# rishabhgoel0213/ZeroClone

Measured on AMD Instinct MI355X. Metric: MCTS node-expansions/sec (whole node), Connect4 800 sims/move at 1/2/4/8 MI355X, higher is better.
Workload: dtype f64

## Files before the change

zeroclone_amd/csrc/c4_device.h:

```cpp
#pragma once
#include <math.h>

#include "c4_order_table.h"
#include "zc_internal.h"

namespace zc {
namespace {

__constant__ uint32_t d_order[128] = {ZC_C4_ORDER_LIST};

constexpr uint32_t kRingMask = kRingWords - 1;
constexpr uint64_t kBottom = 0x0000040810204081ull;
constexpr uint64_t kFull = kBottom * 0x3Full;
constexpr uint64_t kTop = kBottom << 5;
constexpr int kTabBytes = 128 * 4 + 128 * 8;

__device__ __forceinline__ uint32_t untried_init(uint32_t n) { return ((1u << n) - 1u) | (n << 28); }
__device__ __forceinline__ uint32_t untried_count(uint32_t u) { return (uint32_t)__popc(u & 0x7Fu); }

__device__ __forceinline__ void load_tables(uint32_t *s_order) {
    for (int i = (int)threadIdx.x; i < 128; i += blockDim.x) s_order[i] = d_order[i];
    uint8_t *const s_sel = (uint8_t *)(s_order + 128);
    for (int i = (int)threadIdx.x; i < 1024; i += blockDim.x) {
        const uint32_t m = (uint32_t)i >> 3, r = (uint32_t)i & 7u;
// ... 98 lines not shown
    m = b & (b >> 1);
    r |= m & (m >> 2);
    m = b & (b >> 6);
    r |= m & (m >> 12);
    m = b & (b >> 8);
    r |= m & (m >> 16);
    return r != 0;
}

__device__ __forceinline__ uint32_t temper(uint32_t y) {
    y ^= y >> 11;
    y ^= (y << 7) & 0x9d2c5680u;
    y ^= (y << 15) & 0xefc60000u;
    y ^= y >> 18;
    return y;
}

struct Rng {
    uint32_t *ring;
    uint32_t base;
    int32_t wrel;
    uint32_t off;
    int32_t grel;
    uint32_t wt;
    uint32_t wn;
    uint32_t wx;
    __device__ __forceinline__ int32_t use() const { return wrel + (int32_t)off; }
    __device__ __forceinline__ uint32_t slot(int32_t rel) const { return (base + (uint32_t)rel) & kRingMask; }
    __device__ __forceinline__ uint32_t cur() const { return wt; }
};

__device__ __forceinline__ int32_t rng_generate(uint32_t *ring, uint32_t base, int32_t grel, int32_t target) {
    const uint32_t lane = lane_id();
    constexpr int K = kChunk / 64;
    while (grel < target) {
        uint32_t a[K], b[K], m[K];
        const uint32_t p0 = base + (uint32_t)grel + lane;
#pragma unroll
        for (int k = 0; k < K; ++k) {
            const uint32_t p = p0 + 64u * k;
            a[k] = ring[(p - 624) & kRingMask];
            b[k] = ring[(p - 623) & kRingMask];
            m[k] = ring[(p - 227) & kRingMask];
        }
#pragma unroll
        for (int k = 0; k < K; ++k) {
            const uint32_t p = p0 + 64u * k;
            const uint32_t y = (a[k] & 0x80000000u) | (b[k] & 0x7fffffffu);
            ring[p & kRingMask] = m[k] ^ (y >> 1) ^ ((b[k] & 1u) ? 0x9908b0dfu : 0u);
        }
        grel += kChunk;
        wave_mem_order();
    }
    return grel;
}

__device__ __forceinline__ void rng_fill(Rng &r, int32_t target) {
    if (r.grel < target) r.grel = rng_generate(r.ring, r.base, r.grel, target);
}

__device__ __forceinline__ void rng_open(Rng &r, uint32_t *ring, uint64_t use0, uint64_t gen0) {
    r.ring = ring;
    r.base = (uint32_t)use0;
    r.grel = (int32_t)(gen0 - use0);
    r.off = (uint32_t)use0 & (uint32_t)(kWin - 1);
    r.wrel = -(int32_t)r.off;
    rng_fill(r, r.wrel + 3 * kWin);
    r.wt = temper(r.ring[r.slot(r.wrel + (int32_t)lane_id())]);
    r.wn = temper(r.ring[r.slot(r.wrel + kWin + (int32_t)lane_id())]);
    r.wx = r.ring[r.slot(r.wrel + 2 * kWin + (int32_t)lane_id())];
    vmem_ready(r.wx);
}

__device__ __forceinline__ void rng_advance(Rng &r) {
    r.wrel += kWin;
    r.off -= (uint32_t)kWin;
    r.wt = r.wn;
    r.wn = temper(r.wx);
    if (r.grel < r.wrel + 3 * kWin) rng_fill(r, r.wrel + 3 * kWin);
    r.wx = r.ring[r.slot(r.wrel + 2 * kWin + (int32_t)lane_id())];
    vmem_ready(r.wx);
}

template <class R>
__device__ __forceinline__ uint32_t rng_view(const R &r) {
    const uint32_t j = lane_id() + r.off;
    const int idx = (int)(j << 2);
    const uint32_t a = (uint32_t)__builtin_amdgcn_ds_bpermute(idx, (int)r.wt);
    const uint32_t b = (uint32_t)__builtin_amdgcn_ds_bpermute(idx, (int)r.wn);
    return j < 64u ? a : b;
}

__device__ __forceinline__ void rng_close(const Rng &r, uint64_t use0, uint64_t *rngpos) {
    rngpos[0] = use0 + (uint64_t)(int64_t)r.use();
    rngpos[1] = use0 + (uint64_t)(int64_t)r.grel;
}

constexpr int kLRingWords = 1024;
constexpr uint32_t kLRingMask = kLRingWords - 1;
constexpr int kLRingBytes = kLRingWords * 4;

struct LRng {
    uint32_t *lds;
    uint32_t base;
    int32_t wrel;
    uint32_t off;
    int32_t hrel;
    uint32_t wa, wb, ph;
    __device__ __forceinline__ uint32_t cur() const { return ph ? wb : wa; }
    uint32_t wx;
    uint32_t ia, ib, im;
    __device__ __forceinline__ int32_t use() const { return wrel + (int32_t)off; }
    __device__ __forceinline__ uint32_t slot(int32_t rel) const { return (base + (uint32_t)rel) & kLRingMask; }
};

__device__ __forceinline__ uint32_t mt_twist(uint32_t a, uint32_t b, uint32_t m) {
    const uint32_t y = (a & 0x80000000u) | (b & 0x7fffffffu);
    return m ^ (y >> 1) ^ ((b & 1u) ? 0x9908b0dfu : 0u);
}

__device__ __forceinline__ void lrng_prefetch(LRng &r) {
    const int32_t p = r.wrel + 192 + (int32_t)lane_id();
    r.ia = r.lds[r.slot(p - 624)];
    r.ib = r.lds[r.slot(p - 623)];
    r.im = r.lds[r.slot(p - 227)];
}

__device__ __forceinline__ void lrng_generate_abs(uint32_t *lds, uint64_t g, uint64_t end) {
    const uint32_t lane = lane_id();
    for (; g < end; g += 64) {
        const uint32_t p = (uint32_t)g + lane;
        const uint32_t a = lds[(p - 624) & kLRingMask], b = lds[(p - 623) & kLRingMask],
                       m = lds[(p - 227) & kLRingMask];
        if (g + lane < end) lds[p & kLRingMask] = mt_twist(a, b, m);
        wave_mem_order();
    }
}

__device__ __forceinline__ void lrng_open(LRng &r, uint32_t *lds, const uint32_t *ring, uint64_t use0, uint64_t gen0) {
    const uint32_t lane = lane_id();
    r.lds = lds;
    r.base = (uint32_t)use0;
    r.off = (uint32_t)use0 & (uint32_t)(kWin - 1);
    r.wrel = -(int32_t)r.off;
    const uint64_t w0 = use0 - r.off, target = w0 + 192;
    const uint64_t g = gen0 <= w0 + 960 ? gen0 : (target < 624 ? 624 : target);
    for (uint32_t i = lane; i < (uint32_t)kLRingWords; i += 64) {
        const uint32_t p = (uint32_t)g - (uint32_t)kLRingWords + i;
        lds[p & kLRingMask] = ring[p & kRingMask];
    }
    wave_mem_order();
    lrng_generate_abs(lds, g, target);
    r.hrel = (int32_t)(g - use0);
    r.wa = temper(lds[r.slot(r.wrel + (int32_t)lane)]);
    r.wb = temper(lds[r.slot(r.wrel + kWin + (int32_t)lane)]);
    r.ph = 0;
    r.wx = lds[r.slot(r.wrel + 2 * kWin + (int32_t)lane)];
    lrng_prefetch(r);
}

__device__ __forceinline__ uint32_t rng_view(const LRng &r) {
    const uint32_t j = lane_id() + r.off;
    const int idx = (int)(j << 2);
    const uint32_t a = (uint32_t)__builtin_amdgcn_ds_bpermute(idx, (int)r.wa);
    const uint32_t b = (uint32_t)__builtin_amdgcn_ds_bpermute(idx, (int)r.wb);
    return (j ^ r.ph) < 64u ? a : b;
}

__device__ __forceinline__ void rng_advance(LRng &r) {
    r.wrel += kWin;
    r.off -= (uint32_t)kWin;
    const uint32_t t = temper(r.wx);
    if (r.ph) r.wb = t;
    else r.wa = t;
    r.ph ^= 64u;
    const int32_t p = r.wrel + 128 + (int32_t)lane_id();
    uint32_t x = mt_twist(r.ia, r.ib, r.im);
    if (r.wrel + 128 < r.hrel) {
        const uint32_t old = r.lds[r.slot(p)];
        x = p < r.hrel ? old : x;
    }
    r.lds[r.slot(p)] = x;
    r.wx = x;
    lrng_prefetch(r);
}

__device__ __forceinline__ void lrng_skip(LRng &r, uint32_t w) {
    r.off += w;
    while (r.off >= (uint32_t)kWin) rng_advance(r);
}

__device__ __forceinline__ void lrng_close(const LRng &r, uint32_t *ring, uint64_t use0, uint64_t *rngpos) {
    const uint32_t lane = lane_id();
    const uint64_t U = use0 + (uint64_t)(int64_t)r.use();
    uint64_t G = use0 + (uint64_t)(int64_t)max(r.wrel + 192, r.hrel);
    const uint64_t blk = U ? (U - 1) / 624 : 0;
    const uint64_t bend = (blk + 1) * 624;
    wave_mem_order();
    if (G < bend) {
        lrng_generate_abs(r.lds, G, bend);
        G = bend;
    }
    const uint64_t wu = U & ~(uint64_t)(kWin - 1);
    uint64_t start = wu < blk * 624 ? wu : blk * 624;
    start = start < G - 624 ? start : G - 624;
    for (uint64_t q = start + lane; q < G; q += 64) ring[(uint32_t)q & kRingMask] = r.lds[(uint32_t)q & kLRingMask];
    if (lane == 0) {
        rngpos[0] = U;
        rngpos[1] = G;
    }
}

template <class R>
__device__ __forceinline__ uint32_t rng_below(R &r, uint32_t n) {
    const uint32_t sh = (uint32_t)__clz(n);
    const uint32_t lane = lane_id();
    for (;;) {
        if (r.off >= (uint32_t)kWin) rng_advance(r);
        const uint32_t v = r.cur() >> sh;
        const uint64_t bal = __ballot((v | ((lane - r.off) & 0x80000000u)) < n);
        if (bal) {
            const int f = __builtin_ctzll(bal);
            r.off = (uint32_t)f + 1;
            return (uint32_t)__builtin_amdgcn_readlane((int)v, f);
        }
        r.off = kWin;
    }
}

template <class R>
__device__ __forceinline__ uint32_t rng_below_pick(R &r, uint32_t n, const uint8_t *row) {
    const uint32_t sh = (uint32_t)__clz(n);
    const uint32_t lane = lane_id();
    for (;;) {
        if (r.off >= (uint32_t)kWin) rng_advance(r);
        const uint32_t v = r.cur() >> sh;
        const uint32_t pick = row[v & 7u];
        const uint64_t bal = __ballot((v | ((lane - r.off) & 0x80000000u)) < n);
        if (bal) {
            const int f = __builtin_ctzll(bal);
            r.off = (uint32_t)f + 1;
            return (uint32_t)__builtin_amdgcn_readlane((int)pick, f);
        }
        r.off = kWin;
    }
}

struct Counters {
    int32_t expansions = 0, depth_sum = 0, plies = 0, blocks = 0;
    __device__ __forceinline__ void add(int32_t &c, int32_t v) { c += (lane_id() == 0) ? v : 0; }
};

struct Leaf {
    uint64_t p0, p1;
    uint32_t meta;
    int32_t val;
    uint32_t ow;
    uint32_t pad;
};

struct Fresh {
    uint32_t u;
    uint32_t ow;
    uint32_t link;
    uint32_t lmask;
    int32_t na;
    int32_t w;
    uint32_t pad1, pad2;
    uint16_t ch[8];
};
static_assert(sizeof(Fresh) == 48, "Fresh is three 16-byte LDS slots");

struct Tree {
    uint8_t *nodes;
    __device__ __forceinline__ uint8_t *rec(int nd) const { return nodes + (size_t)nd * kRecBytes; }
    __device__ __forceinline__ uint32_t *hdr(int nd) const { return (uint32_t *)rec(nd); }
    __device__ __forceinline__ uint16_t *child(int nd) const { return (uint16_t *)(rec(nd) + 16); }
    __device__ __forceinline__ int32_t *na(int nd) const { return (int32_t *)(rec(nd) + 32); }
    __device__ __forceinline__ double *q(int nd) const { return (double *)(rec(nd) + 64); }
    __device__ __forceinline__ int32_t *w(int nd) const { return (int32_t *)(rec(nd) + 64); }
};

__device__ __forceinline__ void node_init(const Tree &t, int nd, int parent, int pact, int depth, uint32_t ow) {
    const uint32_t lane = lane_id();
    const uint32_t n = (ow >> 24) & 15u;
    if (lane == 0) {
        uint4 h;
        h.x = 0;
        h.y = untried_init(n);
        h.z = (uint32_t)(parent & 0xFFFF) | ((uint32_t)(pact & 0xFF) << 16) | ((uint32_t)depth << 24);
        h.w = ow;
        *(uint4 *)t.rec(nd) = h;
    }
    if (lane < kSlots) {
        t.child(nd)[lane] = 0xFFFF;
        t.na(nd)[lane] = 0;
        t.q(nd)[lane] = 0.0;
    }
}

__device__ __forceinline__ bool valid_state(uint64_t p0, uint64_t p1, int turn) {
    if ((p0 & p1) || ((p0 | p1) & ~kFull) || (turn & ~1)) return false;
    const uint64_t occ = p0 | p1;
#pragma unroll
    for (int c = 0; c < 7; ++c) {
        const uint64_t col = (occ >> (7 * c)) & 0x3Full;
        if (col & (col + 1)) return false;
    }
    return true;
}

template <bool ON>
struct Stamp {
    uint64_t ph[kPhases];
    uint64_t t;
    __device__ __forceinline__ Stamp() : t(ON ? __builtin_amdgcn_s_memtime() : 0) {
        for (int i = 0; i < kPhases; ++i) ph[i] = 0;
    }
    __device__ __forceinline__ void mark(int k) {
        if (ON) {
            const uint64_t now = __builtin_amdgcn_s_memtime();
            ph[k] += now - t;
            t = now;
        }
    }
};

using ConstDouble = const __attribute__((address_space(4))) double;

struct FlushSel {
    int f0;
    int x0node, d0;
    uint32_t ppath;
    bool x0_dirty;
    uint32_t x_u, x_ch;
    bool planned = false;
// ... 262 lines not shown
```

zeroclone_amd/csrc/c4_search.hip:

```cpp
#include "c4_device.h"
#include "counter_rng.h"

namespace zc {
namespace {


__device__ __forceinline__ uint64_t readlane64(uint64_t x, int l) {
    return ((uint64_t)(uint32_t)__builtin_amdgcn_readlane((int)(x >> 32), l) << 32) |
           (uint64_t)(uint32_t)__builtin_amdgcn_readlane((int)x, l);
}

__device__ __forceinline__ uint32_t mbcnt(uint64_t m) {
    return __builtin_amdgcn_mbcnt_hi((uint32_t)(m >> 32), __builtin_amdgcn_mbcnt_lo((uint32_t)m, 0u));
}

__device__ __forceinline__ uint32_t scan_add32(uint32_t x) {
    x += (uint32_t)__builtin_amdgcn_update_dpp(0, (int)x, 0x111, 0xF, 0xF, false);
    x += (uint32_t)__builtin_amdgcn_update_dpp(0, (int)x, 0x112, 0xF, 0xF, false);
    x += (uint32_t)__builtin_amdgcn_update_dpp(0, (int)x, 0x114, 0xF, 0xF, false);
    x += (uint32_t)__builtin_amdgcn_update_dpp(0, (int)x, 0x118, 0xF, 0xF, false);
    x += (uint32_t)__builtin_amdgcn_update_dpp(0, (int)x, 0x142, 0xA, 0xF, false);
    x += (uint32_t)__builtin_amdgcn_update_dpp(0, (int)x, 0x143, 0xC, 0xF, false);
    return x;
}

__device__ __forceinline__ void scan_or16x2(uint32_t &x, uint32_t &y) {
    x |= (uint32_t)__builtin_amdgcn_update_dpp(0, (int)x, 0x111, 0xF, 0xF, false);
    y |= (uint32_t)__builtin_amdgcn_update_dpp(0, (int)y, 0x111, 0xF, 0xF, false);
    x |= (uint32_t)__builtin_amdgcn_update_dpp(0, (int)x, 0x112, 0xF, 0xF, false);
    y |= (uint32_t)__builtin_amdgcn_update_dpp(0, (int)y, 0x112, 0xF, 0xF, false);
    x |= (uint32_t)__builtin_amdgcn_update_dpp(0, (int)x, 0x114, 0xF, 0xF, false);
    y |= (uint32_t)__builtin_amdgcn_update_dpp(0, (int)y, 0x114, 0xF, 0xF, false);
    x |= (uint32_t)__builtin_amdgcn_update_dpp(0, (int)x, 0x118, 0xF, 0xF, false);
    y |= (uint32_t)__builtin_amdgcn_update_dpp(0, (int)y, 0x118, 0xF, 0xF, false);
}

__device__ __forceinline__ uint64_t in_vgpr(uint64_t x) {
    __asm__("" : "+v"(x));
    return x;
}
__device__ __forceinline__ uint32_t ff1(uint64_t m) {
    uint32_t r;
    __asm__("s_ff1_i32_b64 %0, %1" : "=s"(r) : "s"(m));
    return r;
}

#ifndef ZC_RV
#define ZC_RV 0
#endif
#ifndef ZC_LAG_MODE
#define ZC_LAG_MODE 3
#endif
__device__ __forceinline__ void set_prio(int lvl) {
    if (lvl >= 3) __builtin_amdgcn_s_setprio(3);
    else if (lvl == 2) __builtin_amdgcn_s_setprio(2);
    else if (lvl == 1) __builtin_amdgcn_s_setprio(1);
    else __builtin_amdgcn_s_setprio(0);
}
#ifndef ZC_RSTAMP
#define ZC_RSTAMP 0
#endif
#define RMARK(k)                                                    \
    do {                                                            \
        if (ZC_RSTAMP && sub) {                                     \
            __builtin_amdgcn_sched_barrier(0);                      \
            const uint64_t now_ = __builtin_amdgcn_s_memtime();     \
            __builtin_amdgcn_sched_barrier(0);                      \
            if (ZC_RSTAMP == (k)) *sub += now_ - t_;                \
            t_ = now_;                                              \
        }                                                           \
    } while (0)
template <class R>
__device__ void c4_rollouts(Leaf *L, int nb, R &rng, const uint32_t *s_order, Counters &cn,
                            uint64_t *sub = nullptr) {
    uint64_t t_ = ZC_RSTAMP && sub ? __builtin_amdgcn_s_memtime() : 0;
    const uint32_t lane = lane_id();
    const uint32_t lrow = lane >> 4;
    const bool first_row = (lrow & 1u) == 0;
    const uint32_t d1 = lrow < 2 ? 1u : 6u, d2 = lrow < 2 ? 7u : 8u;
    const uint32_t pairbits = lane < 49u ? (1u << (lane / 7u)) | (1u << (lane % 7u)) : 0u;
    for (int g = 0; g < nb; g += 64) {
      uint32_t lm_v = 0, ow_v = 0, hp_v = 0;
      int room_v = 0;
      {
        const int jj = g + (int)lane;
        if (jj < nb) {
            lm_v = L[jj].meta;
            ow_v = L[jj].ow;
            const uint64_t x0 = L[jj].p0, x1 = L[jj].p1;
            const uint64_t op_v = (lm_v >> 24) & 1u ? x0 : x1;
            room_v = has_four(op_v) ? -2 : 41 - __popcll(x0 | x1);
            const uint64_t oc = x0 | x1;
            for (int c = 0; c < 7; ++c) hp_v |= (uint32_t)__popcll((oc >> (7 * c)) & 0x3Full) << (4 * c);
        }
      }
      const int jend = min(nb, g + 64);
      for (int j = g; j < jend; ++j) {
        RMARK(6);
        const int jl = j - g;
        const uint32_t lm = (uint32_t)__builtin_amdgcn_readlane((int)lm_v, jl);
        const uint32_t tnv = (lm >> 24) & 1u;
        const uint64_t *const pp = &L[j].p0;
        uint64_t me = in_vgpr(pp[tnv]);
        uint64_t op = in_vgpr(pp[tnv ^ 1u]);
        uint32_t hp = (uint32_t)__builtin_amdgcn_readlane((int)hp_v, jl);
        const uint32_t low0 = (uint32_t)__builtin_amdgcn_readlane((int)ow_v, jl);
        const int room0 = __builtin_amdgcn_readlane(room_v, jl);
        const bool won = room0 == -2;
        int val = 0;
        int q = 0;
        RMARK(1);
        if (won) {
            val = -1;
        } else if (room0 >= 0) {
            int room = room0;
            int mask = (int)(lm >> 25);
            uint32_t ow = low0;
            uint32_t n = (ow >> 24) & 15u;
            uint32_t sh = (uint32_t)__builtin_clz(n);
            uint32_t owp = s_order[(uint32_t)mask & ~pairbits];
            for (;;) {
                RMARK(6);
                uint32_t wv, v;
                uint64_t A;
                if (rng.off >= (uint32_t)kWin) rng_advance(rng);
                wv = rng_view(rng);
                v = wv >> sh;
                A = __ballot(v < n);
                if (__builtin_expect(A == 0ull, 0)) {
                    do {
                        rng.off += (uint32_t)kWin;
                        rng_advance(rng);
                        wv = rng_view(rng);
                        v = wv >> sh;
                        A = __ballot(v < n);
                    } while (A == 0ull);
                }
#ifndef ZC_DIAG_WASTE
                cn.add(cn.blocks, 1);
#endif
                RMARK(2);
                const uint32_t cap_r = min((uint32_t)room, 30u);
                uint32_t qk = mbcnt(A);
                uint32_t col = (ow >> (3 * v)) & 7u;
                uint32_t one = mask_sel0(A, 1u << (4 * col));
                uint32_t sc = scan_add32(one);
                uint32_t row = ((sc - one + hp) >> (4 * col)) & 15u;
                uint32_t nacc = (uint32_t)__popcll(A);
                uint64_t F = __ballot(row == 5u);
                uint64_t E0 = A & (F | __ballot(qk >= min(cap_r, nacc - 1u)));
                uint32_t l0 = (uint32_t)__builtin_ctzll(E0);
                const uint64_t G = A & F & __ballot(qk < cap_r);
#if !(ZC_RV & 1)
                uint32_t lf = 64u;
                uint32_t cf = 0;
                RMARK(3);
                if (ff1(G) == l0) {
                    lf = l0;
                    cf = (uint32_t)__builtin_amdgcn_readlane((int)col, (int)lf);
                    const uint32_t ow2 = (uint32_t)__builtin_amdgcn_readlane((int)owp, (int)(8u * cf));
                    const uint32_t n2 = (ow2 >> 24) & 15u;
                    const uint32_t v2 = wv >> __clz(n2);
                    const uint64_t low = (2ull << lf) - 1ull;
                    A = (A & low) | (__ballot(v2 < n2) & ~low);
                    qk = mbcnt(A);
                    col = mask_sel(low, (ow2 >> (3 * v2)) & 7u, col);
                    one = mask_sel0(A, 1u << (4 * col));
                    sc = scan_add32(one);
                    row = ((sc - one + hp) >> (4 * col)) & 15u;
                    nacc = (uint32_t)__popcll(A);
                    F = __ballot(row == 5u) & ~low;
                    E0 = A & (F | __ballot(qk >= min(cap_r, nacc - 1u)));
                    l0 = (uint32_t)__builtin_ctzll(E0);
                }
                RMARK(4);
                const uint32_t c = ((qk & 1u) << 4) | ((qk >> 1) & 15u) | (qk & 32u);
                const uint32_t b = __umul24(col, 7u) + row;
                const uint32_t pl = (uint32_t)__builtin_amdgcn_ds_permute((int)(mask_sel(A, 63u, c) << 2), (int)b);
                const uint32_t pb = __builtin_amdgcn_permlane32_swap(pl, pl, false, false)[0];
                const uint64_t bit = 1ull << (pb & 63u);
                uint32_t blo = (uint32_t)bit, bhi = (uint32_t)(bit >> 32);
                scan_or16x2(blo, bhi);
                const uint64_t mine = ((uint64_t)bhi << 32) | blo;
                const uint64_t bd = (first_row ? me : op) | mine;
                const uint64_t m1 = bd & (bd >> d1), m2 = bd & (bd >> d2);
                const uint64_t f4 = (m1 & (m1 >> (2 * d1))) | (m2 & (m2 >> (2 * d2)));
                const uint64_t W = __ballot(f4 != 0ull);
                const uint32_t W32 = (uint32_t)W | (uint32_t)(W >> 32);
                const uint64_t Ew = A & __ballot(((W32 >> (c & 31u)) & 1u) != 0u);
#else
                uint32_t lf = 64u;
                uint32_t cf = 0;
                auto win_test = [&](uint64_t A_, uint32_t qk_, uint32_t col_, uint32_t row_, uint64_t &mine_) {
                    const uint32_t c = ((qk_ & 1u) << 4) | ((qk_ >> 1) & 15u) | (qk_ & 32u);
                    const uint32_t b = __umul24(col_, 7u) + row_;
                    const uint32_t pl = (uint32_t)__builtin_amdgcn_ds_permute((int)(mask_sel(A_, 63u, c) << 2), (int)b);
                    const uint32_t pb = __builtin_amdgcn_permlane32_swap(pl, pl, false, false)[0];
                    const uint64_t bit = 1ull << (pb & 63u);
                    uint32_t blo = (uint32_t)bit, bhi = (uint32_t)(bit >> 32);
                    scan_or16x2(blo, bhi);
                    mine_ = ((uint64_t)bhi << 32) | blo;
                    const uint64_t bd = (first_row ? me : op) | mine_;
                    const uint64_t m1 = bd & (bd >> d1), m2 = bd & (bd >> d2);
                    const uint64_t f4 = (m1 & (m1 >> (2 * d1))) | (m2 & (m2 >> (2 * d2)));
                    const uint64_t W = __ballot(f4 != 0ull);
                    const uint32_t W32 = (uint32_t)W | (uint32_t)(W >> 32);
                    return A_ & __ballot(((W32 >> (c & 31u)) & 1u) != 0u);
                };
                uint64_t Ew1 = 0, mine1 = 0;
                RMARK(3);
                if (ff1(G) == l0) {
                    lf = l0;
                    cf = (uint32_t)__builtin_amdgcn_readlane((int)col, (int)lf);
                    const uint32_t ow2 = (uint32_t)__builtin_amdgcn_readlane((int)owp, (int)(8u * cf));
                    const uint32_t n2 = (ow2 >> 24) & 15u;
                    const uint32_t v2 = wv >> __clz(n2);
                    const uint64_t low = (2ull << lf) - 1ull;
                    if (ZC_RV & 1) Ew1 = win_test(A, qk, col, row, mine1) & low;
                    A = (A & low) | (__ballot(v2 < n2) & ~low);
                    qk = mbcnt(A);
                    col = mask_sel(low, (ow2 >> (3 * v2)) & 7u, col);
                    one = mask_sel0(A, 1u << (4 * col));
                    sc = scan_add32(one);
                    row = ((sc - one + hp) >> (4 * col)) & 15u;
                    nacc = (uint32_t)__popcll(A);
                    F = __ballot(row == 5u) & ~low;
                    E0 = A & (F | __ballot(qk >= min(cap_r, nacc - 1u)));
                    l0 = (uint32_t)__builtin_ctzll(E0);
                }
                RMARK(4);
                uint64_t mine, Ew;
                if ((ZC_RV & 1) && Ew1 != 0ull) {
                    Ew = Ew1;
                    mine = mine1;
                } else {
                    Ew = win_test(A, qk, col, row, mine);
                }
#endif
                const uint32_t ew = ff1(Ew);
                const uint32_t endlane = min(ew, l0);
                const bool win = ew <= l0;
                const uint32_t endply = (uint32_t)__builtin_amdgcn_readlane((int)qk, (int)endlane);
                rng.off += endlane + 1u;
#ifdef ZC_DIAG_WASTE
                cn.add(cn.blocks, lf < 64u && endlane < lf ? 1 : 0);
                cn.add(cn.plies, lf < 64u ? 1 : 0);
#endif
                room -= (int)endply + 1;
                RMARK(5);
                if (win) {
                    val = ((room0 - room) & 1) ? 1 : -1;
                    break;
                }
                if (room < 0) {
                    val = 0;
                    break;
                }
                {
                    const uint64_t s2 = readlane64(mine, (int)((endply + 31u) >> 1));
                    const uint64_t a2 = me | readlane64(mine, (int)(endply >> 1));
                    const uint64_t b2 = op | (endply ? s2 : 0ull);
                    const bool odd = endply & 1u;
                    me = odd ? a2 : b2;
                    op = odd ? b2 : a2;
                }
                hp += (uint32_t)__builtin_amdgcn_readlane((int)sc, (int)endlane);
                const bool fa = endlane >= lf;
                const bool fe = (F >> endlane) & 1u;
                {
                    const uint32_t ce = fe ? (uint32_t)__builtin_amdgcn_readlane((int)col, (int)endlane) : cf;
                    const uint32_t ca = fa ? cf : ce;
                    const bool ff = fa | fe;
                    mask = ff ? mask & ~((1 << ca) | (1 << ce)) : mask;
                    const uint32_t ownew = (uint32_t)__builtin_amdgcn_readlane((int)owp, (int)((7u * ca + ce) & 63u));
                    ow = ff ? ownew : ow;
                    owp = s_order[(uint32_t)mask & ~pairbits];
                }
                n = (ow >> 24) & 15u;
                sh = (uint32_t)__builtin_clz(n);
            }
            q = room0 - room;
        }
        L[j].val = val;
#ifndef ZC_DIAG_WASTE
        cn.add(cn.plies, q);
#endif
      }
    }
}

__device__ void c4_rollouts_philox(Leaf *L, int nb, const uint8_t *s_sel, uint2 key, uint32_t leaf0, uint32_t tag,
                                   uint32_t game, Counters &cn) {
    const uint32_t lane = lane_id();
    for (int base = 0; base < nb; base += kBlock) {
        const int j = base + (int)lane;
        int val = 0, q = 0;
        if (j < nb) {
            const uint64_t x0 = L[j].p0, x1 = L[j].p1;
            const bool tn = (L[j].meta >> 24) & 1u;
            uint64_t me = tn ? x1 : x0;
            uint64_t op = tn ? x0 : x1;
            int stones = __popcll(me | op);
            if (has_four(op)) {
                val = -1;
            } else if (stones < 42) {
                uint32_t legal = (uint32_t)legal_mask(me | op);
                const uint4 sd = philox(make_uint4(leaf0 + (uint32_t)j, tag, game, 0x0C4F0A57u), key);
                Xoshiro128 x{sd.x | ((sd.x | sd.y | sd.z | sd.w) == 0u), sd.y, sd.z, sd.w};
                for (;;) {
                    const uint32_t n = (uint32_t)__popc(legal);
                    const uint32_t k = __umulhi(x.next(), n);
                    const uint32_t col = s_sel[legal * 8u + k];
                    const uint32_t h = (uint32_t)__popcll(((me | op) >> (7u * col)) & 0x3Full);
                    me |= 1ull << (7u * col + h);
                    ++q;
                    ++stones;
                    if (h == 5u) legal &= ~(1u << col);
                    if (has_four(me)) {
                        val = (q & 1) ? 1 : -1;
                        break;
                    }
                    if (stones == 42) {
                        val = 0;
                        break;
                    }
                    const uint64_t t = me;
                    me = op;
                    op = t;
                }
            }
            L[j].val = val;
        }
        int tot = q;
        for (int o = 32; o > 0; o >>= 1) tot += __shfl_xor(tot, o);
        cn.add(cn.plies, tot);
    }
}

struct ChainNode {
    uint64_t p0, p1;
    uint32_t ow;
    uint32_t info;
    uint32_t ul;
    uint32_t pad;
};
static_assert(sizeof(ChainNode) == 32, "chain table entry");

__device__ __forceinline__ uint64_t lanes_in(int lo, int hi) {
    const uint64_t below_hi = hi >= 64 ? ~0ull : (1ull << hi) - 1ull;
    return below_hi & ~((1ull << lo) - 1ull);
}

__device__ __forceinline__ WalkEnd walk_hbm_prefetch(const Tree &t, ConstDouble *logtab, uint64_t rp0, uint64_t rp1,
                                                     int rturn, int done, double c, int &status) {
    const uint32_t lane = lane_id();
    const uint32_t k = lane & 7u, cs = lane >> 3;
    int node = 0, depth = 0, turn = rturn, nN = done;
    uint64_t b0 = rp0, b1 = rp1;
    uint32_t pathv = (lane == 0) ? 0x00FF0000u : 0u;
    const uint8_t *R0 = t.rec(0);
    uint32_t u = uni(((const uint32_t *)R0)[1]), ow = uni(((const uint32_t *)R0)[3]);
    uint32_t ch = ((const uint16_t *)(R0 + 16))[k];
    int32_t na = ((const int32_t *)(R0 + 32))[k];
    int32_t wa = ((const int32_t *)(R0 + 64))[k];
    for (;;) {
        if (untried_count(u)) break;
        if (depth >= kMaxDepth - 2) {
            status = ZC_STATUS_INTERNAL;
            u = 0;
            break;
// ... 714 lines not shown
                        uint8_t *R = t.rec(f0 + r);
                        if (slot == 0) *(uint4 *)R = make_uint4(0u, F.u, F.link, F.ow);
                        ((uint16_t *)(R + 16))[slot] = c;
                        ((int32_t *)(R + 32))[slot] = na;
                        ((int32_t *)(R + 64))[slot] = w;
                    }
                }
            }
        }
        wave_mem_order();
        stamp.mark(6);
        done += nb;
        if (stop && done < p.sims && status == 0 && uni(spent) >= budget) break;
        if (ZC_LAG_MODE >= 2 && progress) {
            const int64_t own = ((int64_t)mv * p.sims + done) * p.n_games, avg = (int64_t)spent * p.sims;
            const int64_t mvn = (int64_t)p.sims * p.n_games;
            if (ZC_LAG_MODE == 4)
                lag = own >= avg ? 0 : own + mvn / 2 > avg ? 1 : own + mvn > avg ? 2 : 3;
            else
                lag = own < avg ? (ZC_LAG_MODE == 3 && own + mvn <= avg ? 2 : ZC_LAG_MODE == 3 ? 1 : 2) : 0;
            set_prio(lag);
        }
    }
    done_io = done;
    nnodes_io = nnodes;
    if (lagp) *lagp = lag;
    if (STAMP && lane == 0)
        for (int k_ = 0; k_ < kPhases; ++k_) p.a.phase[kPhases * (size_t)g + k_] += (int64_t)stamp.ph[k_];
}

__device__ __forceinline__ int best_column(const Tree &t, int &na_col) {
    const uint32_t lane = lane_id();
    const uint32_t k = lane & 7u;
    const uint32_t u = uni(t.hdr(0)[1]);
    const uint32_t ow = uni(t.hdr(0)[3]);
    const uint32_t nm = u >> 28;
    int bv = (k < nm) ? t.na(0)[k] : -1;
    int bi = (int)k;
    argmax8(bv, bi);
    const int best = uni(bi);
    int pos = -1;
    for (uint32_t s = 0; s < nm; ++s)
        if (((ow >> (3 * s)) & 7u) == lane) pos = (int)s;
    na_col = pos >= 0 ? t.na(0)[pos] : 0;
    return (int)((ow >> (3 * best)) & 7u);
}

template <bool STAMP, bool PHILOX, int WALK>
__device__ __forceinline__ void search_games(const SearchParams &p, uint8_t *s_dyn) {
    const SearchLds L = search_lds(s_dyn, p.bs);
    load_tables(L.s_order);
    __syncthreads();

    const uint32_t lane = lane_id();
    const int gl = (int)(blockIdx.x * (blockDim.x >> 6) + (threadIdx.x >> 6));
    if (gl >= p.n_games) return;
    const int g = p.game_ids ? uni(p.game_ids[gl]) : p.first_game + gl;
    {
        const zc_c4_state root = p.roots[gl];
        const uint64_t rp0 = uni64(root.stones[0]), rp1 = uni64(root.stones[1]);
        const int rturn = uni(root.turn);
        if (!valid_state(rp0, rp1, rturn) || legal_mask(rp0 | rp1) == 0) {
            if (lane == 0) {
                zc_game_stats st{};
                st.status = valid_state(rp0, rp1, rturn) ? ZC_STATUS_NO_MOVES : ZC_STATUS_BAD_STATE;
                p.out_stats[gl] = st;
                p.out_move[gl] = -1;
            }
            if (lane < 7) p.out_na[(size_t)gl * 7 + lane] = 0;
            return;
        }
    }
    const Arena &a = p.a;
    const Tree t{a.nodes + (size_t)g * p.M * kRecBytes};
    LRng rng;
    const uint64_t use0 = uni64(a.rngpos[2 * (size_t)g]);
    lrng_open(rng, L.ring, a.ring + (size_t)g * kRingWords, use0, uni64(a.rngpos[2 * (size_t)g + 1]));
    Counters cn;
    int status = 0, done = 0, nnodes = 1;
    search_move<STAMP, PHILOX, WALK>(p, L, gl, g, t, rng, uni((uint32_t)use0), cn, status, done, nnodes);
    int na_col;
    const int col = best_column(t, na_col);
    if (lane < 7) p.out_na[(size_t)gl * 7 + lane] = na_col;
    if (lane == 0) {
        p.out_move[gl] = col;
        zc_game_stats st{};
        st.status = status;
        st.expansions = cn.expansions;
        st.depth_sum = cn.depth_sum;
        st.leaves = p.sims;
        st.rollout_plies = cn.plies;
        st.rollout_blocks = cn.blocks;
        st.rng_words = rng.use();
        p.out_stats[gl] = st;
    }
    lrng_close(rng, a.ring + (size_t)g * kRingWords, use0, a.rngpos + 2 * (size_t)g);
}

template <bool STAMP, bool PHILOX>
__global__ __launch_bounds__(kSearchWaves * kBlock, 4) void c4_search_kernel(SearchParams p) {
    extern __shared__ __attribute__((aligned(16))) uint8_t s_dyn[];
    search_games<STAMP, PHILOX, 0>(p, s_dyn);
}

template <int WALK>
__global__ __launch_bounds__(kSearchWaves * kBlock, 4) void c4_walk_kernel(SearchParams p) {
    extern __shared__ __attribute__((aligned(16))) uint8_t s_dyn[];
    search_games<false, false, WALK>(p, s_dyn);
}

template <bool PHILOX>
__global__ __launch_bounds__(kSearchWaves * kBlock, 4) void c4_selfplay_kernel(SearchParams p) {
    extern __shared__ __attribute__((aligned(16))) uint8_t s_dyn[];
    const SearchLds L = search_lds(s_dyn, p.bs);
    load_tables(L.s_order);
    __syncthreads();

    const uint32_t lane = lane_id();
    const int gl = (int)(blockIdx.x * (blockDim.x >> 6) + (threadIdx.x >> 6));
    if (gl >= p.n_games) return;
    const int g = p.first_game + gl;
    const Arena &a = p.a;
    const Tree t{a.nodes + (size_t)g * p.M * kRecBytes};
    LRng rng;
    const uint64_t use0 = uni64(a.rngpos[2 * (size_t)g]);
    lrng_open(rng, L.ring, a.ring + (size_t)g * kRingWords, use0, uni64(a.rngpos[2 * (size_t)g + 1]));
    Counters cn;
    int status = 0;
    int finished = 0;
    int mv = 0;
    int64_t leaves = 0;
    uint64_t t_start = 0, t_last = 0;
    if (p.tstamps) t_start = t_last = __builtin_amdgcn_s_memrealtime();
    int lag = 0;
    uint4 cy = a.carry[g];
    cy = make_uint4(uni(cy.x), uni(cy.y), uni(cy.z), 0u);
    bool resume = cy.x != 0;
    for (; mv < p.moves; ++mv) {
        if (p.ticket && !resume) {
            int tk = 0;
            if (lane == 0) tk = atomicAdd(p.ticket, 1);
            if (uni(tk) >= p.budget) break;
        }
        if (p.tstamps) t_last = __builtin_amdgcn_s_memrealtime();
        zc_c4_state root = p.roots[gl];
        uint64_t s0 = uni64(root.stones[0]), s1 = uni64(root.stones[1]);
        int turn = uni(root.turn);
        if (!valid_state(s0, s1, turn) || legal_mask(s0 | s1) == 0) {
            status = ZC_STATUS_BAD_STATE;
            break;
        }
        int done = resume ? (int)cy.x : 0, nnodes = resume ? (int)cy.y : 1;
        const uint32_t tag = resume ? cy.z : uni((uint32_t)(use0 + (uint64_t)(int64_t)rng.use()));
        const int done0 = done;
        if (ZC_LAG_MODE == 1 && p.progress) {
            const int32_t tot = __hip_atomic_load(p.progress, __ATOMIC_RELAXED, __HIP_MEMORY_SCOPE_AGENT);
            lag = (int64_t)mv * p.n_games < (int64_t)uni(tot) ? 2 : 0;
            set_prio(lag);
        }
        search_move<false, PHILOX>(p, L, gl, g, t, rng, tag, cn, status, done, nnodes, p.carry ? p.ticket : nullptr,
                                   p.budget, &lag, ZC_LAG_MODE ? p.progress : nullptr, mv);
        if (ZC_LAG_MODE && p.progress && lane == 0) atomicAdd(p.progress, 1);
        leaves += done - done0;
        if (done < p.sims) {
            if (lane == 0) a.carry[g] = make_uint4((uint32_t)done, (uint32_t)nnodes, tag, 0u);
            break;
        }
        if (resume && lane == 0) a.carry[g] = make_uint4(0u, 0u, 0u, 0u);
        resume = false;
        int na_col;
        const int col = best_column(t, na_col);
        const uint64_t bit = drop_bit(s0 | s1, col);
        if (turn) s1 |= bit; else s0 |= bit;
        const bool won = has_four(turn ? s1 : s0);
        turn ^= 1;
        const int r = won ? turn * 2 - 1 : ((s0 | s1) == kFull ? 0 : ZC_C4_ONGOING);
        const size_t o = (size_t)mv * p.n_games + gl;
        if (lane == 0) {
            zc_c4_state post;
            post.stones[0] = s0;
            post.stones[1] = s1;
            post.turn = turn;
            post.reserved = 0;
            p.out_states[o] = post;
            p.out_moves16[o] = (int16_t)col;
            p.out_results[o] = r;
            p.io_roots[gl] = r == ZC_C4_ONGOING ? post : zc_c4_state{{0, 0}, 0, 0};
        }
        finished += r != ZC_C4_ONGOING;
        wave_mem_order();
    }
    if (p.ticket && lane == 0) atomicMax(p.ticket + 1, mv);
    if (p.tstamps && lane == 0) {
        uint64_t *ts = p.tstamps + 4 * (size_t)g;
        ts[0] = t_start;
        ts[1] = t_last;
        ts[2] = __builtin_amdgcn_s_memrealtime();
        const uint32_t hw = (uint32_t)__builtin_amdgcn_s_getreg(4 | (15 << 11)) |
                            ((uint32_t)__builtin_amdgcn_s_getreg(20 | (3 << 11)) << 16);
        ts[3] = (uint64_t)mv | ((uint64_t)hw << 32);
    }
    for (int k = mv + (int)lane; k < p.moves; k += kBlock) {
        const size_t o = (size_t)k * p.n_games + gl;
        p.out_moves16[o] = -1;
        p.out_results[o] = ZC_SLOT_SKIP;
    }
    if (lane == 0) {
        zc_game_stats st{};
        st.status = status;
        st.expansions = cn.expansions;
        st.depth_sum = cn.depth_sum;
        st.leaves = leaves;
        st.rollout_plies = cn.plies;
        st.rollout_blocks = cn.blocks;
        st.rng_words = rng.use();
        st.reserved = finished;
        p.out_stats[gl] = st;
    }
    lrng_close(rng, a.ring + (size_t)g * kRingWords, use0, a.rngpos + 2 * (size_t)g);
}

__global__ __launch_bounds__(kBlock) void c4_rollout_debug_kernel(Arena a, int first_game, int n,
                                                                  const zc_c4_state *states, int32_t *out_value,
                                                                  int64_t *out_words) {
    __shared__ Leaf s_leaf[1];
    __shared__ uint32_t s_order[kTabBytes / 4];
    load_tables(s_order);
    __syncthreads();
    const uint32_t lane = lane_id();
    const int gl = blockIdx.x;
    if (gl >= n) return;
    const int g = first_game + gl;
    Rng rng;
    const uint64_t use0 = uni64(a.rngpos[2 * (size_t)g]);
    rng_open(rng, a.ring + (size_t)g * kRingWords, use0, uni64(a.rngpos[2 * (size_t)g + 1]));
    const zc_c4_state s = states[gl];
    if (lane == 0) {
        s_leaf[0].p0 = s.stones[0];
        s_leaf[0].p1 = s.stones[1];
        s_leaf[0].meta = ((uint32_t)s.turn << 24) | ((uint32_t)legal_mask(s.stones[0] | s.stones[1]) << 25);
        s_leaf[0].ow = s_order[legal_mask(s.stones[0] | s.stones[1])];
    }
    wave_mem_order();
    Counters cn;
    c4_rollouts(s_leaf, 1, rng, s_order, cn);
    wave_mem_order();
    if (lane == 0) {
        out_value[gl] = s_leaf[0].val;
        out_words[gl] = rng.use();
        rng_close(rng, use0, a.rngpos + 2 * (size_t)g);
    }
}

__global__ __launch_bounds__(kBlock) void c4_rollout_seq_kernel(Arena a, int g, int n, const zc_c4_state *states,
                                                                int32_t *out_value, int64_t *out_words) {
    __shared__ Leaf s_leaf[kBlock];
    __shared__ uint32_t s_order[kTabBytes / 4];
    load_tables(s_order);
    __syncthreads();
    const uint32_t lane = lane_id();
    Rng rng;
    const uint64_t use0 = uni64(a.rngpos[2 * (size_t)g]);
    rng_open(rng, a.ring + (size_t)g * kRingWords, use0, uni64(a.rngpos[2 * (size_t)g + 1]));
    Counters cn;
    for (int base = 0; base < n; base += kBlock) {
        const int cnt = min(kBlock, n - base);
        if ((int)lane < cnt) {
            const zc_c4_state s = states[base + lane];
            s_leaf[lane].p0 = s.stones[0];
            s_leaf[lane].p1 = s.stones[1];
            s_leaf[lane].meta = ((uint32_t)s.turn << 24) | ((uint32_t)legal_mask(s.stones[0] | s.stones[1]) << 25);
            s_leaf[lane].ow = s_order[legal_mask(s.stones[0] | s.stones[1])];
        }
        wave_mem_order();
        rng_fill(rng, rng.use() + kLookahead);
        c4_rollouts(s_leaf, cnt, rng, s_order, cn);
        wave_mem_order();
        if ((int)lane < cnt) out_value[base + lane] = s_leaf[lane].val;
        wave_mem_order();
    }
    if (lane == 0) {
        out_words[0] = rng.use();
        rng_close(rng, use0, a.rngpos + 2 * (size_t)g);
    }
}

__global__ void c4_play_kernel(int n, zc_c4_state *states, const int32_t *moves, int32_t *results, int reset) {
    const int i = blockIdx.x * blockDim.x + threadIdx.x;
    if (i >= n) return;
    const int col = moves[i];
    if (col < 0 || col > 6) {
        results[i] = ZC_C4_ONGOING;
        return;
    }
    zc_c4_state s = states[i];
    const int turn = s.turn & 1;
    s.stones[turn] |= drop_bit(s.stones[0] | s.stones[1], col);
// ... 98 lines not shown
```

Before: 3.252 billion.

## Streamline rollout inner loop: single bpermute rng view, mask-select boards, batched leaf stores

rng_view now selects the source register per lane before a single ds_bpermute, where it used to issue two bpermutes and then select. The LRng phase becomes a 64-bit lane mask so window updates are branchless mask selects. In the rollout loop, each leaf is loaded as one 16-byte vector and the boards are kept as x0/x1 with a lane-mask side selector instead of swapping me/op. The block loop is restructured with a scalar compare-select exit test. Per-leaf value and ply writes are collected via writelane and stored once per 64-leaf group. Counter accumulation moves to per-lane sums that are reduced at the end, which adds shuffle reductions and more complex control flow.

```diff
diff --git a/zeroclone_amd/csrc/c4_device.h b/zeroclone_amd/csrc/c4_device.h
--- a/zeroclone_amd/csrc/c4_device.h
+++ b/zeroclone_amd/csrc/c4_device.h
@@ -204,13 +204,10 @@
     vmem_ready(r.wx);
 }
 
-template <class R>
-__device__ __forceinline__ uint32_t rng_view(const R &r) {
-    const uint32_t j = lane_id() + r.off;
-    const int idx = (int)(j << 2);
-    const uint32_t a = (uint32_t)__builtin_amdgcn_ds_bpermute(idx, (int)r.wt);
-    const uint32_t b = (uint32_t)__builtin_amdgcn_ds_bpermute(idx, (int)r.wn);
-    return j < 64u ? a : b;
+__device__ __forceinline__ uint32_t rng_view(const Rng &r) {
+    const uint32_t lane = lane_id();
+    const uint32_t src = lane < r.off ? r.wn : r.wt;
+    return (uint32_t)__builtin_amdgcn_ds_bpermute((int)((lane + r.off) << 2), (int)src);
 }
 
 __device__ __forceinline__ void rng_close(const Rng &r, uint64_t use0, uint64_t *rngpos) {
@@ -228,8 +225,9 @@
     int32_t wrel;
     uint32_t off;
     int32_t hrel;
-    uint32_t wa, wb, ph;
-    __device__ __forceinline__ uint32_t cur() const { return ph ? wb : wa; }
+    uint32_t wa, wb;
+    uint64_t ph;
+    __device__ __forceinline__ uint32_t cur() const { return mask_sel(ph, wa, wb); }
     uint32_t wx;
     uint32_t ia, ib, im;
     __device__ __forceinline__ int32_t use() const { return wrel + (int32_t)off; }
@@ -282,20 +280,19 @@
 }
 
 __device__ __forceinline__ uint32_t rng_view(const LRng &r) {
-    const uint32_t j = lane_id() + r.off;
-    const int idx = (int)(j << 2);
-    const uint32_t a = (uint32_t)__builtin_amdgcn_ds_bpermute(idx, (int)r.wa);
-    const uint32_t b = (uint32_t)__builtin_amdgcn_ds_bpermute(idx, (int)r.wb);
-    return (j ^ r.ph) < 64u ? a : b;
+    const uint32_t lane = lane_id();
+    const uint32_t src = mask_sel(__ballot(lane < r.off) ^ r.ph, r.wa, r.wb);
+    return (uint32_t)__builtin_amdgcn_ds_bpermute((int)((lane + r.off) << 2), (int)src);
 }
 
 __device__ __forceinline__ void rng_advance(LRng &r) {
     r.wrel += kWin;
     r.off -= (uint32_t)kWin;
     const uint32_t t = temper(r.wx);
-    if (r.ph) r.wb = t;
-    else r.wa = t;
-    r.ph ^= 64u;
+    const uint32_t na = mask_sel(r.ph, t, r.wa), nb = mask_sel(r.ph, r.wb, t);
+    r.wa = na;
+    r.wb = nb;
+    r.ph = ~r.ph;
     const int32_t p = r.wrel + 128 + (int32_t)lane_id();
     uint32_t x = mt_twist(r.ia, r.ib, r.im);
     if (r.wrel + 128 < r.hrel) {
@@ -371,9 +368,13 @@
 struct Counters {
     int32_t expansions = 0, depth_sum = 0, plies = 0, blocks = 0;
     __device__ __forceinline__ void add(int32_t &c, int32_t v) { c += (lane_id() == 0) ? v : 0; }
-};
-
-struct Leaf {
+    __device__ __forceinline__ static int32_t total(int32_t c) {
+        for (int o = 32; o; o >>= 1) c += __shfl_xor(c, o);
+        return c;
+    }
+};
+
+struct alignas(16) Leaf {
     uint64_t p0, p1;
     uint32_t meta;
     int32_t val;
diff --git a/zeroclone_amd/csrc/c4_search.hip b/zeroclone_amd/csrc/c4_search.hip
--- a/zeroclone_amd/csrc/c4_search.hip
+++ b/zeroclone_amd/csrc/c4_search.hip
@@ -39,6 +39,12 @@
     __asm__("" : "+v"(x));
     return x;
 }
+__device__ __forceinline__ int neg_if_le(uint32_t a, uint32_t b, int y) {
+    int r;
+    __asm__("s_cmp_le_u32 %1, %2\n\ts_cselect_b32 %0, -1, %3" : "=s"(r) : "s"(a), "s"(b), "s"(y) : "scc");
+    return r;
+}
+extern "C" __device__ int zc_writelane(int x, int l, int old) __asm("llvm.amdgcn.writelane.i32");
 __device__ __forceinline__ uint32_t ff1(uint64_t m) {
     uint32_t r;
     __asm__("s_ff1_i32_b64 %0, %1" : "=s"(r) : "s"(m));
@@ -76,12 +82,14 @@
     uint64_t t_ = ZC_RSTAMP && sub ? __builtin_amdgcn_s_memtime() : 0;
     const uint32_t lane = lane_id();
     const uint32_t lrow = lane >> 4;
-    const bool first_row = (lrow & 1u) == 0;
+    const uint64_t second_rows = __ballot((lrow & 1u) != 0);
     const uint32_t d1 = lrow < 2 ? 1u : 6u, d2 = lrow < 2 ? 7u : 8u;
     const uint32_t pairbits = lane < 49u ? (1u << (lane / 7u)) | (1u << (lane % 7u)) : 0u;
+    __builtin_amdgcn_s_waitcnt(0x0F70);
     for (int g = 0; g < nb; g += 64) {
       uint32_t lm_v = 0, ow_v = 0, hp_v = 0;
       int room_v = 0;
+      int val_v = 0, q_v = 0;
       {
         const int jj = g + (int)lane;
         if (jj < nb) {
@@ -92,6 +100,9 @@
             room_v = has_four(op_v) ? -2 : 41 - __popcll(x0 | x1);
             const uint64_t oc = x0 | x1;
             for (int c = 0; c < 7; ++c) hp_v |= (uint32_t)__popcll((oc >> (7 * c)) & 0x3Full) << (4 * c);
+#ifndef ZC_DIAG_WASTE
+            cn.blocks += room_v >= 0 ? 1 : 0;
+#endif
         }
       }
       const int jend = min(nb, g + 64);
@@ -99,27 +110,26 @@
         RMARK(6);
         const int jl = j - g;
         const uint32_t lm = (uint32_t)__builtin_amdgcn_readlane((int)lm_v, jl);
-        const uint32_t tnv = (lm >> 24) & 1u;
-        const uint64_t *const pp = &L[j].p0;
-        uint64_t me = in_vgpr(pp[tnv]);
-        uint64_t op = in_vgpr(pp[tnv ^ 1u]);
+        uint4 pw;
+        __builtin_memcpy(&pw, &L[j], sizeof pw);
+        uint64_t x0 = ((uint64_t)pw.y << 32) | pw.x, x1 = ((uint64_t)pw.w << 32) | pw.z;
+        uint64_t S1 = (lm >> 24) & 1u ? ~second_rows : second_rows;
         uint32_t hp = (uint32_t)__builtin_amdgcn_readlane((int)hp_v, jl);
         const uint32_t low0 = (uint32_t)__builtin_amdgcn_readlane((int)ow_v, jl);
         const int room0 = __builtin_amdgcn_readlane(room_v, jl);
-        const bool won = room0 == -2;
-        int val = 0;
+        int val = (room0 + 1) >> 1;
         int q = 0;
         RMARK(1);
-        if (won) {
-            val = -1;
-        } else if (room0 >= 0) {
+        if (room0 >= 0) {
             int room = room0;
             int mask = (int)(lm >> 25);
             uint32_t ow = low0;
             uint32_t n = (ow >> 24) & 15u;
             uint32_t sh = (uint32_t)__builtin_clz(n);
             uint32_t owp = s_order[(uint32_t)mask & ~pairbits];
-            for (;;) {
+            uint32_t ew, l0, lf, endlane, endply, col, sc;
+            uint64_t F, mine;
+            auto block = [&]() __attribute__((always_inline)) {
                 RMARK(6);
                 uint32_t wv, v;
                 uint64_t A;
@@ -136,40 +146,38 @@
                         A = __ballot(v < n);
                     } while (A == 0ull);
                 }
-#ifndef ZC_DIAG_WASTE
-                cn.add(cn.blocks, 1);
-#endif
                 RMARK(2);
                 const uint32_t cap_r = min((uint32_t)room, 30u);
                 uint32_t qk = mbcnt(A);
-                uint32_t col = (ow >> (3 * v)) & 7u;
+                col = (ow >> (3 * v)) & 7u;
                 uint32_t one = mask_sel0(A, 1u << (4 * col));
-                uint32_t sc = scan_add32(one);
+                sc = scan_add32(one);
                 uint32_t row = ((sc - one + hp) >> (4 * col)) & 15u;
                 uint32_t nacc = (uint32_t)__popcll(A);
-                uint64_t F = __ballot(row == 5u);
+                F = __ballot(row == 5u);
                 uint64_t E0 = A & (F | __ballot(qk >= min(cap_r, nacc - 1u)));
-                uint32_t l0 = (uint32_t)__builtin_ctzll(E0);
+                l0 = (uint32_t)__builtin_ctzll(E0);
                 const uint64_t G = A & F & __ballot(qk < cap_r);
+                lf = ff1(G);
+#ifdef ZC_DIAG_WASTE
+                const uint32_t l0f = l0;
+#endif
 #if !(ZC_RV & 1)
-                uint32_t lf = 64u;
-                uint32_t cf = 0;
                 RMARK(3);
-                if (ff1(G) == l0) {
-                    lf = l0;
-                    cf = (uint32_t)__builtin_amdgcn_readlane((int)col, (int)lf);
+                if (lf == l0) {
+                    const uint32_t cf = (uint32_t)__builtin_amdgcn_readlane((int)col, (int)lf);
                     const uint32_t ow2 = (uint32_t)__builtin_amdgcn_readlane((int)owp, (int)(8u * cf));
                     const uint32_t n2 = (ow2 >> 24) & 15u;
                     const uint32_t v2 = wv >> __clz(n2);
-                    const uint64_t low = (2ull << lf) - 1ull;
-                    A = (A & low) | (__ballot(v2 < n2) & ~low);
+                    const uint64_t high = ~1ull << lf;
+                    A = (A & ~high) | (__ballot(v2 < n2) & high);
                     qk = mbcnt(A);
-                    col = mask_sel(low, (ow2 >> (3 * v2)) & 7u, col);
+                    col = mask_sel(high, col, (ow2 >> (3 * v2)) & 7u);
                     one = mask_sel0(A, 1u << (4 * col));
                     sc = scan_add32(one);
                     row = ((sc - one + hp) >> (4 * col)) & 15u;
                     nacc = (uint32_t)__popcll(A);
-                    F = __ballot(row == 5u) & ~low;
+                    F = __ballot(row == 5u) & high;
                     E0 = A & (F | __ballot(qk >= min(cap_r, nacc - 1u)));
                     l0 = (uint32_t)__builtin_ctzll(E0);
                 }
@@ -181,16 +189,17 @@
                 const uint64_t bit = 1ull << (pb & 63u);
                 uint32_t blo = (uint32_t)bit, bhi = (uint32_t)(bit >> 32);
                 scan_or16x2(blo, bhi);
-                const uint64_t mine = ((uint64_t)bhi << 32) | blo;
-                const uint64_t bd = (first_row ? me : op) | mine;
+                mine = ((uint64_t)bhi << 32) | blo;
+                x0 = in_vgpr(x0);
+                x1 = in_vgpr(x1);
+                const uint64_t bd = (((uint64_t)mask_sel(S1, (uint32_t)(x0 >> 32), (uint32_t)(x1 >> 32)) << 32) |
+                                     mask_sel(S1, (uint32_t)x0, (uint32_t)x1)) | mine;
                 const uint64_t m1 = bd & (bd >> d1), m2 = bd & (bd >> d2);
                 const uint64_t f4 = (m1 & (m1 >> (2 * d1))) | (m2 & (m2 >> (2 * d2)));
                 const uint64_t W = __ballot(f4 != 0ull);
                 const uint32_t W32 = (uint32_t)W | (uint32_t)(W >> 32);
                 const uint64_t Ew = A & __ballot(((W32 >> (c & 31u)) & 1u) != 0u);
 #else
-                uint32_t lf = 64u;
-                uint32_t cf = 0;
                 auto win_test = [&](uint64_t A_, uint32_t qk_, uint32_t col_, uint32_t row_, uint64_t &mine_) {
                     const uint32_t c = ((qk_ & 1u) << 4) | ((qk_ >> 1) & 15u) | (qk_ & 32u);
                     const uint32_t b = __umul24(col_, 7u) + row_;
@@ -200,7 +209,10 @@
                     uint32_t blo = (uint32_t)bit, bhi = (uint32_t)(bit >> 32);
                     scan_or16x2(blo, bhi);
                     mine_ = ((uint64_t)bhi << 32) | blo;
-                    const uint64_t bd = (first_row ? me : op) | mine_;
+                    x0 = in_vgpr(x0);
+                    x1 = in_vgpr(x1);
+                    const uint64_t bd = (((uint64_t)mask_sel(S1, (uint32_t)(x0 >> 32), (uint32_t)(x1 >> 32)) << 32) |
+                                         mask_sel(S1, (uint32_t)x0, (uint32_t)x1)) | mine_;
                     const uint64_t m1 = bd & (bd >> d1), m2 = bd & (bd >> d2);
                     const uint64_t f4 = (m1 & (m1 >> (2 * d1))) | (m2 & (m2 >> (2 * d2)));
                     const uint64_t W = __ballot(f4 != 0ull);
@@ -209,67 +221,65 @@
                 };
                 uint64_t Ew1 = 0, mine1 = 0;
                 RMARK(3);
-                if (ff1(G) == l0) {
-                    lf = l0;
-                    cf = (uint32_t)__builtin_amdgcn_readlane((int)col, (int)lf);
+                if (lf == l0) {
+                    const uint32_t cf = (uint32_t)__builtin_amdgcn_readlane((int)col, (int)lf);
                     const uint32_t ow2 = (uint32_t)__builtin_amdgcn_readlane((int)owp, (int)(8u * cf));
                     const uint32_t n2 = (ow2 >> 24) & 15u;
                     const uint32_t v2 = wv >> __clz(n2);
-                    const uint64_t low = (2ull << lf) - 1ull;
-                    if (ZC_RV & 1) Ew1 = win_test(A, qk, col, row, mine1) & low;
-                    A = (A & low) | (__ballot(v2 < n2) & ~low);
+                    const uint64_t high = ~1ull << lf;
+                    if (ZC_RV & 1) Ew1 = win_test(A, qk, col, row, mine1) & ~high;
+                    A = (A & ~high) | (__ballot(v2 < n2) & high);
                     qk = mbcnt(A);
-                    col = mask_sel(low, (ow2 >> (3 * v2)) & 7u, col);
+                    col = mask_sel(high, col, (ow2 >> (3 * v2)) & 7u);
                     one = mask_sel0(A, 1u << (4 * col));
                     sc = scan_add32(one);
                     row = ((sc - one + hp) >> (4 * col)) & 15u;
                     nacc = (uint32_t)__popcll(A);
-                    F = __ballot(row == 5u) & ~low;
+                    F = __ballot(row == 5u) & high;
                     E0 = A & (F | __ballot(qk >= min(cap_r, nacc - 1u)));
                     l0 = (uint32_t)__builtin_ctzll(E0);
                 }
                 RMARK(4);
-                uint64_t mine, Ew;
+                uint64_t Ew;
                 if ((ZC_RV & 1) && Ew1 != 0ull) {
                     Ew = Ew1;
                     mine = mine1;
                 } else {
                     Ew = win_test(A, qk, col, row, mine);
                 }
+                if (ZC_RV & 1) Ew = uni64(Ew);
 #endif
-                const uint32_t ew = ff1(Ew);
-                const uint32_t endlane = min(ew, l0);
-                const bool win = ew <= l0;
-                const uint32_t endply = (uint32_t)__builtin_amdgcn_readlane((int)qk, (int)endlane);
+                ew = ff1(Ew);
+                endlane = min(ew, l0);
+                endply = (uint32_t)__builtin_amdgcn_readlane((int)qk, (int)endlane);
                 rng.off += endlane + 1u;
 #ifdef ZC_DIAG_WASTE
-                cn.add(cn.blocks, lf < 64u && endlane < lf ? 1 : 0);
-                cn.add(cn.plies, lf < 64u ? 1 : 0);
+                cn.add(cn.blocks, lf == l0f && endlane < lf ? 1 : 0);
+                cn.add(cn.plies, lf == l0f ? 1 : 0);
 #endif
                 room -= (int)endply + 1;
                 RMARK(5);
-                if (win) {
-                    val = ((room0 - room) & 1) ? 1 : -1;
-                    break;
-                }
-                if (room < 0) {
-                    val = 0;
-                    break;
-                }
+                return neg_if_le(ew, l0, room);
+            };
+            auto go_on = [&]() __attribute__((always_inline)) {
+#ifndef ZC_DIAG_WASTE
+                cn.add(cn.blocks, 1);
+#endif
                 {
                     const uint64_t s2 = readlane64(mine, (int)((endply + 31u) >> 1));
-                    const uint64_t a2 = me | readlane64(mine, (int)(endply >> 1));
-                    const uint64_t b2 = op | (endply ? s2 : 0ull);
-                    const bool odd = endply & 1u;
-                    me = odd ? a2 : b2;
-                    op = odd ? b2 : a2;
+                    const uint64_t a2 = readlane64(mine, (int)(endply >> 1));
+                    const uint64_t b2 = endply ? s2 : 0ull;
+                    const bool p1_first = S1 & 1ull;
+                    x0 |= p1_first ? b2 : a2;
+                    x1 |= p1_first ? a2 : b2;
+                    S1 = endply & 1u ? S1 : ~S1;
                 }
                 hp += (uint32_t)__builtin_amdgcn_readlane((int)sc, (int)endlane);
                 const bool fa = endlane >= lf;
                 const bool fe = (F >> endlane) & 1u;
                 {
-                    const uint32_t ce = fe ? (uint32_t)__builtin_amdgcn_readlane((int)col, (int)endlane) : cf;
-                    const uint32_t ca = fa ? cf : ce;
+                    const uint32_t ca = (uint32_t)__builtin_amdgcn_readlane((int)col, (int)(fa ? lf : endlane));
+                    const uint32_t ce = fe ? (uint32_t)__builtin_amdgcn_readlane((int)col, (int)endlane) : ca;
                     const bool ff = fa | fe;
                     mask = ff ? mask & ~((1 << ca) | (1 << ce)) : mask;
                     const uint32_t ownew = (uint32_t)__builtin_amdgcn_readlane((int)owp, (int)((7u * ca + ce) & 63u));
@@ -278,14 +288,21 @@
                 }
                 n = (ow >> 24) & 15u;
                 sh = (uint32_t)__builtin_clz(n);
+            };
+            if (block() >= 0) {
+                do go_on();
+                while (block() >= 0);
             }
             q = room0 - room;
-        }
-        L[j].val = val;
+            val = ew <= l0 ? ((q & 1) ? 1 : -1) : 0;
+        }
+        val_v = zc_writelane(val, jl, val_v);
+        q_v = zc_writelane(q, jl, q_v);
+      }
+      if (g + (int)lane < jend) L[g + (int)lane].val = val_v;
 #ifndef ZC_DIAG_WASTE
-        cn.add(cn.plies, q);
+      cn.plies += q_v;
 #endif
-      }
     }
 }
 
@@ -1166,6 +1183,7 @@
     int na_col;
     const int col = best_column(t, na_col);
     if (lane < 7) p.out_na[(size_t)gl * 7 + lane] = na_col;
+    const int32_t plies = Counters::total(cn.plies), blocks = Counters::total(cn.blocks);
     if (lane == 0) {
         p.out_move[gl] = col;
         zc_game_stats st{};
@@ -1173,8 +1191,8 @@
         st.expansions = cn.expansions;
         st.depth_sum = cn.depth_sum;
         st.leaves = p.sims;
-        st.rollout_plies = cn.plies;
-        st.rollout_blocks = cn.blocks;
+        st.rollout_plies = plies;
+        st.rollout_blocks = blocks;
         st.rng_words = rng.use();
         p.out_stats[gl] = st;
     }
@@ -1289,14 +1307,15 @@
         p.out_moves16[o] = -1;
         p.out_results[o] = ZC_SLOT_SKIP;
     }
+    const int32_t plies = Counters::total(cn.plies), blocks = Counters::total(cn.blocks);
     if (lane == 0) {
         zc_game_stats st{};
         st.status = status;
         st.expansions = cn.expansions;
         st.depth_sum = cn.depth_sum;
         st.leaves = leaves;
-        st.rollout_plies = cn.plies;
-        st.rollout_blocks = cn.blocks;
+        st.rollout_plies = plies;
+        st.rollout_blocks = blocks;
         st.rng_words = rng.use();
         st.reserved = finished;
         p.out_stats[gl] = st;
```

Measured after the change: 3.428 billion, median of 6. 1.05x the previous value.
